# MLCogUP/nspeech

Measured on AMD Instinct MI355X. Metric: mel-frames/sec Tacotron-2 LJSpeech bs32 train step, higher is better.
Workload: dtype bf16; 1 GPU; Tacotron-2 train step (fwd+bwd+clip+Adam), batch 32/GPU, T_in 160, T_out 1000, r=5; targets = spectrogram features of synthetic speech (SURVEY 8d); global_batch=32, parallelism=dp1, deterministic_gradients=True

## Files before the change

### include/nspeech_hip.h

```cpp
#ifndef NSPEECH_HIP_H
#define NSPEECH_HIP_H
#include <stddef.h>
#include <stdint.h>

#ifdef __cplusplus
extern "C" {
#endif

typedef void* ns_stream_t;

enum { NS_OK = 0, NS_ERR_BAD_ARG = -1, NS_ERR_UNSUPPORTED_SHAPE = -2, NS_ERR_LAUNCH = -3,
       NS_ERR_SHORT_BUFFER = -4  };
enum { NS_F32 = 0, NS_BF16 = 1, NS_F64 = 2  };
enum { NS_ACT_NONE = 0, NS_ACT_RELU = 1, NS_ACT_TANH = 2, NS_ACT_SIGMOID = 3,
       NS_ACT_SOFTSIGN = 4  };

int ns_version(void);
const char* ns_device_arch(void);
const char* ns_last_error(void);

int ns_occupy(int blocks, int threads, int lds_bytes, int heavy, double usec, int* started, ns_stream_t stream);
int ns_wait_counter(const int* counter, int target, double timeout_usec, ns_stream_t stream);

typedef struct {
  float count, eps, momentum;
  int training;
  float* moving_mean; float* moving_var;
  float* mean_out; float* istd_out;
} ns_gemm_bn_params;
typedef struct {
  int dtype;
  int M, N, K;
  const void* A; int64_t lda; int a_mode;
  const void* B; int64_t ldb; int b_mode;
  int b_seg_len; int64_t b_seg_stride;
  void* C; int64_t ldc; int c_dtype;
  int accumulate;
  const float* bias;
  int act;
  float alpha;
  int row_period, row_lo, row_hi, row_shift;
  float* col_sum; float* col_sumsq;
  int split_k;
  const void* addend; int64_t ld_add;
  const void* gate; int64_t ld_gate;
  int f32_passes;
  int addend_dtype;
  const void* A_lo; const void* B_lo;
  int batch; int64_t batch_stride_a, batch_stride_b, batch_stride_c;
  float* stat_part;
  int stat_slots;
  const void* stat_z; int64_t ld_stat_z; int stat_z_dtype;
  const float* stat_mean; const float* stat_istd;
  float* splitk_work; int* splitk_count;
  ns_gemm_bn_params bn;
} ns_gemm_params;
int ns_gemm(const ns_gemm_params* p, ns_stream_t stream);
size_t ns_gemm_stat_part_floats(int M, int N);
size_t ns_gemm_splitk_work_bytes(int M, int N, int split_k);
size_t ns_gemm_splitk_counters(int M, int N);
const char* ns_gemm_last_kernel(void);



typedef struct {
  const void* src; int src_dtype; int64_t src_si, src_sj;
  void* dst; int dst_dtype; int64_t dst_si, dst_sj;
  int I, J, Cc;
  int accumulate;
} ns_copy3d_params;
int ns_copy3d(const ns_copy3d_params* p, ns_stream_t stream);

typedef struct {
  const int* ids;
  const float* table;
  void* out; int out_dtype;
  int N, T, P, padl, D, V;
} ns_embedding_params;
int ns_embedding_fwd(const ns_embedding_params* p, ns_stream_t stream);
typedef struct {
  const int* ids;
  const float* dout;
  float* dtable;
  int N, T, P, padl, D, V;
  float* work;
} ns_embedding_bwd_params;
int ns_embedding_bwd(const ns_embedding_bwd_params* p, ns_stream_t stream);
size_t ns_embedding_bwd_work_floats(int N, int D, int V);

typedef struct {
  const void* z; void* y; int dtype;
  int rows, C;
  const float* col_sum; const float* col_sumsq; float count;
  const float* gamma; const float* beta;
  float* moving_mean; float* moving_var;
  float* mean_out; float* istd_out;
  float eps, momentum;
  int training;
  int row_period, row_lo, row_hi;
  void* y_hi; void* y_lo;
  int64_t ld_y;
  int stats_final;
} ns_bn_fwd_params;
int ns_bn_fwd(const ns_bn_fwd_params* p, ns_stream_t stream);

typedef struct {
  const float* dy; const void* z; void* dpre; int dtype;
  int rows, C;
  const float* mean; const float* istd; const float* gamma;
  float* dgamma; float* dbeta; float* dbias;
  float* work;
  float count;
  int act;
  int row_period, row_lo, row_hi;
// ... 491 lines not shown
```

### nspeech_amd/csrc/gemm.hip

```cpp
#include "common.h"
#include "colsum4.h"
#include <limits.h>

struct Epi {
  void* C; long ldc; int c_dtype; int accumulate;
  const float* bias; int act; float alpha;
  int row_period, row_lo, row_hi, row_shift;
  int M, N;
  const void* addend; long ld_add; int add_bf16;
  const void* gate; long ld_gate; int gate_dtype;
  const void* sz; long ld_sz; int sz_bf16; const float* smean; const float* sistd;
};

__device__ __forceinline__ Epi make_epi(const ns_gemm_params& p) {
  Epi e;
  e.C = p.C; e.ldc = p.ldc; e.c_dtype = p.c_dtype; e.accumulate = p.accumulate;
  e.bias = p.bias; e.act = p.act; e.alpha = p.alpha;
  e.row_period = p.row_period; e.row_lo = p.row_lo; e.row_hi = p.row_hi; e.row_shift = p.row_shift;
  e.M = p.M; e.N = p.N;
  e.addend = p.addend; e.ld_add = p.ld_add; e.add_bf16 = p.addend_dtype == NS_BF16;
  e.gate = p.gate; e.ld_gate = p.ld_gate; e.gate_dtype = p.dtype;
  e.sz = p.stat_z; e.ld_sz = p.ld_stat_z; e.sz_bf16 = p.stat_z_dtype == NS_BF16; e.smean = p.stat_mean; e.sistd = p.stat_istd;
  return e;
}
// ... 197 lines not shown
    for (int j = 0; j < 4; ++j) { As[ty][tx * 4 + j] = s1[j]; Bs[ty][tx * 4 + j] = s2[j]; }
    __syncthreads();
    if (tid < BN && n0 + tid < p.N) {
      float a = 0.f, b = 0.f;
      for (int r = 0; r < 16; ++r) { a += As[r][tid]; b += Bs[r][tid]; }
      p.stat_part[(long)blockIdx.y * p.N + n0 + tid] = a;
      p.stat_part[((long)p.stat_slots + blockIdx.y) * p.N + n0 + tid] = b;
    }
  }
}

__global__ __launch_bounds__(1024) void gemm_stats_finalize_kernel(const float* part, int slots, int N, float* col_sum,
                                                                   float* col_sumsq, ns_gemm_bn_params bn) {
  __shared__ float red[32][33][2];
  const int c = threadIdx.x & 31, q = threadIdx.x >> 5;
  const int n = blockIdx.x * 32 + c;
  float a = 0.f, b = 0.f;
  if (n < N) {
    for (int s = q; s < slots; s += 32) {
      a += part[(long)s * N + n];
      b += part[((long)slots + s) * N + n];
    }
  }
  red[q][c][0] = a; red[q][c][1] = b;
  __syncthreads();
#pragma unroll
  for (int h = 16; h >= 1; h >>= 1) {
    if (q < h) { red[q][c][0] += red[q + h][c][0]; red[q][c][1] += red[q + h][c][1]; }
    __syncthreads();
  }
  if (q == 0 && n < N) {
    col_sum[n] = red[0][c][0];
    if (col_sumsq) col_sumsq[n] = red[0][c][1];
    if (bn.mean_out)
      bn_finalize_column(n, red[0][c][0], red[0][c][1], bn.count, bn.eps, bn.momentum, bn.training, bn.moving_mean,
                         bn.moving_var, bn.mean_out, bn.istd_out);
  }
}

constexpr int GBM = 128, GBN = 128, GBK = 64;

__device__ __forceinline__ int row_img_off(int row, int chunk) {
  return row * 128 + ((chunk ^ ((row >> 1) & 7)) << 4);
}
__device__ __forceinline__ int col_swz(int k) { return (k & 3) | ((k >> 1) & 4); }
__device__ __forceinline__ int col_img_off_chunk(int k, int chunk) {
  return k * 256 + ((chunk ^ (col_swz(k) << 1)) << 4);
}
__device__ __forceinline__ int col_img_off_unit(int k, int unit) {
  return k * 256 + ((unit ^ (col_swz(k) << 2)) << 3);
}

typedef __attribute__((address_space(3))) bf16x4 lds_bf16x4;

__device__ __forceinline__ bf16x8 frag_row(const char* img, int row, int chunk) {
  return *(const bf16x8*)(img + row_img_off(row, chunk));
}
__device__ __forceinline__ bf16x8 frag_col(const char* img, int kbase, int col0, int lane) {
  const int i16 = lane & 15, g = lane >> 4;
  const int q = i16 >> 2, pp = i16 & 3;
  const int k = kbase + 8 * g + q;
  const int unit = (col0 >> 2) + pp;
  bf16x4 t0 = __builtin_amdgcn_ds_read_tr16_b64_v4bf16((lds_bf16x4*)(img + col_img_off_unit(k, unit)));
  bf16x4 t1 = __builtin_amdgcn_ds_read_tr16_b64_v4bf16((lds_bf16x4*)(img + col_img_off_unit(k + 4, unit)));
  return __builtin_shufflevector(t0, t1, 0, 1, 2, 3, 4, 5, 6, 7);
}

struct Stage { uint4 v[4]; };

template <int MODE, int BK = GBK, int ROWS = 128>
__device__ __forceinline__ void stage_load(Stage& s, const bf16_t* base, long ld, int r0, int extent,
                                           int k0, int K, int tid) {
  if (MODE == 0) {
    const int c = tid & 7;
#pragma unroll
    for (int i = 0; i < ROWS / 32; ++i) {
      const int row = (tid >> 3) + 32 * i;
      const int r = r0 + row, k = k0 + c * 8;
      if (r < extent && k < K) s.v[i] = *(const uint4*)(base + (long)r * ld + k);
      else s.v[i] = make_uint4(0, 0, 0, 0);
    }
  } else {
    const int c = tid & 15;
#pragma unroll
    for (int i = 0; i < BK / 16; ++i) {
      const int kr = (tid >> 4) + 16 * i;
      const int k = k0 + kr, r = r0 + c * 8;
      if (k < K && r < extent) s.v[i] = *(const uint4*)(base + (long)k * ld + r);
      else s.v[i] = make_uint4(0, 0, 0, 0);
    }
  }
}
template <int MODE, int BK = GBK, int ROWS = 128>
__device__ __forceinline__ void stage_store(const Stage& s, char* img, int tid) {
  if (MODE == 0) {
    const int c = tid & 7;
#pragma unroll
    for (int i = 0; i < ROWS / 32; ++i) {
      const int row = (tid >> 3) + 32 * i;
      *(uint4*)(img + row_img_off(row, c)) = s.v[i];
    }
  } else {
    const int c = tid & 15;
#pragma unroll
    for (int i = 0; i < BK / 16; ++i) {
      const int kr = (tid >> 4) + 16 * i;
// ... 197 lines not shown
    char* imgB = imgA + IMG;
    const bool more = kt + 1 < kt1;
    if (more) {
      int kin;
      const bf16_t* bb = b_tile_base((kt + 1) * BK, kin);
      stage_load<AMODE, BK, TM>(sa, A, p.lda, m0, p.M, (kt + 1) * BK, p.K, tid);
      stage_load<BMODE, BK>(sb, bb, p.ldb, n0, p.N, kin, KB, tid);
    }
#pragma unroll
    for (int ks = 0; ks < BK / 32; ++ks) {
      bf16x8 af[4], bfr[NJ];
#pragma unroll
      for (int i = 0; i < 4; ++i) {
        if (AMODE == 0) af[i] = frag_row(imgA, wm * 64 + i * 16 + (lane & 15), ks * 4 + (lane >> 4));
        else af[i] = frag_col(imgA, ks * 32, wm * 64 + i * 16, lane);
      }
#pragma unroll
      for (int j = 0; j < NJ; ++j) {
        if (BMODE == 0) bfr[j] = frag_row(imgB, wn * (NJ * 16) + j * 16 + (lane & 15), ks * 4 + (lane >> 4));
        else bfr[j] = frag_col(imgB, ks * 32, wn * (NJ * 16) + j * 16, lane);
      }
#pragma unroll
      for (int i = 0; i < 4; ++i)
#pragma unroll
        for (int j = 0; j < NJ; ++j)
          acc[i][j] = VEC ? __builtin_amdgcn_mfma_f32_16x16x32_bf16(bfr[j], af[i], acc[i][j], 0, 0, 0)
                          : __builtin_amdgcn_mfma_f32_16x16x32_bf16(af[i], bfr[j], acc[i][j], 0, 0, 0);
    }
    if (more) {
      char* nA = smem + (cur ^ 1) * 2 * IMG;
      stage_store<AMODE, BK, TM>(sa, nA, tid);
      stage_store<BMODE, BK>(sb, nA + IMG, tid);
    }
    __syncthreads();
  }

  bool add_bias = ksl == 0;
  if (p.splitk_work && p.split_k > 1) {
    if (!splitk_gather_acc<NJ>(p, acc, wgid, ksl, tid)) return;
    add_bias = true;
  }
  if constexpr (VEC) x256_quadrant(p, acc, m0 + wm * 64, n0 + wn * (NJ * 16), lane);
  else mfma_epilogue(p, acc, m0, n0, wm, wn, lane, add_bias);
}
template <int AMODE, int BMODE, bool VEC, int BK = GBK, int TM = GBM>
__global__ __launch_bounds__(256, BK == 64 ? 2 : 3) void gemm_mfma_kernel(ns_gemm_params p) {
  const int nwg = ((p.M + TM - 1) / TM) * ((p.N + GBN - 1) / GBN);
  int wgid, ksl;
  xcd_work_item(p, nwg, wgid, ksl);
  batch_shift(p, blockIdx.z);
  gemm_mfma_body<AMODE, BMODE, VEC, BK, TM>(p, wgid, ksl);
}

constexpr int XHALF = 16384, XBUF = 65536;

typedef __attribute__((address_space(1))) const void* gptr_t;
typedef __attribute__((address_space(3))) void* lptr_t;

template <int NSEG>
__global__ __launch_bounds__(512, 1) void gemm_x256_kernel(ns_gemm_params p) {
  extern __shared__ __attribute__((aligned(1024))) char smem[];
  const int tid = threadIdx.x, lane = tid & 63;
  const int wave = __builtin_amdgcn_readfirstlane(tid >> 6);
  const int wr = wave >> 2, wc = wave & 3;
  const int tiles_n = (p.N + 255) / 256, tiles_m = (p.M + 255) / 256;
  const int nwg = tiles_m * tiles_n;
  int wgid;
  {
    const int orig = blockIdx.x, xcd = orig & 7, q = nwg >> 3, r = nwg & 7;
    wgid = (xcd < r ? xcd * (q + 1) : r * (q + 1) + (xcd - r) * q) + (orig >> 3);
  }
  const int tm = wgid / tiles_n, tn = wgid % tiles_n;
  const int m0 = tm * 256, n0 = tn * 256;
  const int nk = p.K / 64, NT = nk * NSEG;

  unsigned offA00, offA01, offA10, offA11, offB00, offB01, offB10, offB11;
  {
    const int r0 = wave * 8 + (lane >> 3), r1 = r0 + 64;
    const int c0 = (lane & 7) ^ ((r0 >> 1) & 7), c1 = (lane & 7) ^ ((r1 >> 1) & 7);
    auto oa = [&](int h, int r, int c) { return (unsigned)(((long)min(m0 + h * 128 + r, p.M - 1) * p.lda + c * 8) * 2); };
    auto ob = [&](int h, int r, int c) { return (unsigned)(((long)min(n0 + h * 128 + r, p.N - 1) * p.ldb + c * 8) * 2); };
    offA00 = oa(0, r0, c0); offA01 = oa(0, r1, c1); offA10 = oa(1, r0, c0); offA11 = oa(1, r1, c1);
    offB00 = ob(0, r0, c0); offB01 = ob(0, r1, c1); offB10 = ob(1, r0, c0); offB11 = ob(1, r1, c1);
  }
  const char* const Ahi = (const char*)p.A;
  const char* const Bhi = (const char*)p.B;
  const char* const Alo = (const char*)p.A_lo;
  const char* const Blo = (const char*)p.B_lo;
  char* const lstage = smem + wave * 1024;

#define X_ISSUE(T, HALF, O0, O1, ISA)                                                                   \
  do {                                                                                                   \
    const int t_ = (T);                                                                                  \
    if (t_ < NT) {                                                                                       \
      const int sg_ = NSEG == 1 ? 0 : t_ / nk;                                                           \
      const int kt_ = NSEG == 1 ? t_ : t_ - sg_ * nk;                                                    \
      const char* g_ = (ISA) ? (sg_ == NSEG - 1 && NSEG > 1 ? Alo : Ahi) : (sg_ == 1 && NSEG == 3 ? Blo : Bhi); \
      if (!(ISA) && p.b_seg_len > 0) {       \
        const int bs_ = (kt_ * 64) / p.b_seg_len;                                                        \
        g_ += ((long)bs_ * p.b_seg_stride + (kt_ * 64 - bs_ * p.b_seg_len)) * 2;                         \
      } else {                                                                                           \
        g_ += (long)kt_ * 128;                                                                           \
      }                                                                                                  \
      char* l_ = lstage + (t_ & 1) * XBUF + (HALF) * XHALF;                                              \
      __builtin_amdgcn_global_load_lds((gptr_t)(g_ + (O0)), (lptr_t)l_, 16, 0, 0);                       \
      __builtin_amdgcn_global_load_lds((gptr_t)(g_ + (O1)), (lptr_t)(l_ + 8192), 16, 0, 0);             \
    }                                                                                                    \
  } while (0)
#define X_ISSUE_A0(T) X_ISSUE(T, 0, offA00, offA01, 1)
#define X_ISSUE_A1(T) X_ISSUE(T, 1, offA10, offA11, 1)
// ... 370 lines not shown

template <int PASSES, int MT, int NC>
__global__ __launch_bounds__(SKW * 64) void gemm_skinny_f32_kernel(ns_gemm_params p) {
  __shared__ float red[SKW][16 * MT][20];
  const int tid = threadIdx.x, lane = tid & 63, wave = tid >> 6;
  const int n0 = blockIdx.x * NC;
  const int m0 = blockIdx.y * 16 * MT;
  const float* A = (const float*)p.A;
  const float* B = (const float*)p.B;
  const int r16 = lane & 15, g = lane >> 4;
  f32x4 acc[MT];
#pragma unroll
  for (int i = 0; i < MT; ++i) acc[i] = (f32x4){0.f, 0.f, 0.f, 0.f};
  const int nkc = (p.K + 31) / 32;
  const bool ok0 = m0 + r16 < p.M, ok1 = MT > 1 && m0 + 16 + r16 < p.M, okn = r16 < NC && n0 + r16 < p.N;
  for (int kc0 = wave; kc0 < nkc; kc0 += SKW * 2) {
    bf16x8 ah[2][MT], al[2][MT], bh[2], bl[2];
#pragma unroll
    for (int q = 0; q < 2; ++q) {
      const int k = (kc0 + q * SKW) * 32 + g * 8;
      const bool okk = k < p.K;
      ldsplit8(A + (long)(m0 + r16) * p.lda + k, ok0 && okk, ah[q][0], al[q][0]);
      if (MT > 1) ldsplit8(A + (long)(m0 + 16 + r16) * p.lda + k, ok1 && okk, ah[q][MT - 1], al[q][MT - 1]);
      ldsplit8(B + (long)(n0 + r16) * p.ldb + k, okn && okk, bh[q], bl[q]);
    }
#pragma unroll
    for (int q = 0; q < 2; ++q)
#pragma unroll
      for (int i = 0; i < MT; ++i) acc[i] = mfma_split<PASSES>(ah[q][i], al[q][i], bh[q], bl[q], acc[i]);
  }
#pragma unroll
  for (int i = 0; i < MT; ++i)
#pragma unroll
    for (int r = 0; r < 4; ++r) red[wave][i * 16 + g * 4 + r][r16] = acc[i][r];
  __syncthreads();
  Epi e = make_epi(p);
  for (int idx = tid; idx < 16 * MT * NC; idx += SKW * 64) {
    const int mm = idx / NC, nn = idx % NC;
    const int m = m0 + mm, n = n0 + nn;
    if (m >= p.M || n >= p.N) continue;
    float v = 0.f;
#pragma unroll
    for (int w = 0; w < SKW; ++w) v += red[w][mm][nn];
    const bool valid = row_valid(e, m);
    v = epi_value(e, m, n, v, true, valid);
    epi_store(e, m, n, v);
  }
}

static bool aligned16(const void* p) { return (((uintptr_t)p) & 15) == 0; }

static thread_local const char* g_last_kernel = "";
extern "C" const char* ns_gemm_last_kernel(void) { return g_last_kernel; }

static bool vec_epilogue_ok(const ns_gemm_params& p) {
  auto al = [](const void* q, long ld, bool bf16) { return !q || ((((uintptr_t)q) & (bf16 ? 7 : 15)) == 0 && ld % 4 == 0); };
  if (p.accumulate == 2 || p.split_k != 1 || p.N % 4 != 0) return false;
  if (p.batch > 1 && p.batch_stride_c % 4 != 0) return false;
  return al(p.C, p.ldc, p.c_dtype == NS_BF16) && al(p.addend, p.ld_add, p.addend_dtype == NS_BF16) &&
         al(p.gate, p.ld_gate, p.dtype == NS_BF16) && al(p.stat_z, p.ld_stat_z, p.stat_z_dtype == NS_BF16) &&
         al(p.bias, 4, false) && al(p.stat_mean, 4, false) && al(p.stat_istd, 4, false) && al(p.stat_part, 4, false);
}
static bool half_tiles_wanted(const ns_gemm_params& p, int tiles128) {
  static const int env = [] { const char* e = getenv("NS_GEMM_HALF"); return e ? atoi(e) : -1; }();
  if (env == 0 || env == 1) return env != 0;
  return tiles128 * p.batch <= (env > 1 ? env : 256) && p.M > 64;
}
static bool x256_ok(const ns_gemm_params& p) {
  if (p.dtype != NS_BF16 || p.a_mode != 0 || p.b_mode != 0 || p.split_k != 1) return false;
  if (p.b_seg_len != 0 && (p.b_seg_len % 64 != 0 || p.b_seg_stride % 8 != 0)) return false;
  if (p.K % 64 != 0 || p.K < 128 || p.M < 1024 || p.N % 128 != 0) return false;
  if ((p.A_lo != nullptr) != (p.B_lo != nullptr)) return false;
  if (p.A_lo && (!aligned16(p.A_lo) || !aligned16(p.B_lo))) return false;
  {
    auto al = [](const void* q, long ld, bool bf16) { return !q || ((((uintptr_t)q) & (bf16 ? 7 : 15)) == 0 && ld % 4 == 0); };
    if (!al(p.C, p.ldc, p.c_dtype == NS_BF16) || !al(p.addend, p.ld_add, p.addend_dtype == NS_BF16) ||
        !al(p.gate, p.ld_gate, true) || !al(p.stat_z, p.ld_stat_z, p.stat_z_dtype == NS_BF16) || !al(p.bias, 4, false) ||
        !al(p.stat_mean, 4, false) || !al(p.stat_istd, 4, false) || !al(p.stat_part, 4, false)) return false;
  }
  if ((double)p.M * (double)p.lda * 2.0 >= 4.0e9 || (double)p.N * (double)p.ldb * 2.0 >= 4.0e9) return false;
  if (getenv("NS_GEMM_NO256")) return false;
  return ceil_div(p.M, 256) * ceil_div(p.N, 256) >= 96;
}

extern "C" size_t ns_gemm_stat_part_floats(int M, int N) {
  if (M <= 0 || N <= 0) return 0;
  return (size_t)2 * 4 * ceil_div(M, 256) * (size_t)N;
}

static int gemm_dispatch(ns_gemm_params& p, hipStream_t stream);

int ns_stats_finalize(const float* part, int slots, int N, float* s1, float* s2, hipStream_t stream) {
  hipLaunchKernelGGL(gemm_stats_finalize_kernel, dim3(ceil_div(N, 32)), dim3(1024), 0, stream, part, slots, N, s1, s2,
                     ns_gemm_bn_params{});
  NS_CHECK_LAUNCH("gemm_stats_finalize");
  return NS_OK;
}

extern "C" size_t ns_gemm_splitk_work_bytes(int M, int N, int split_k) {
  if (split_k <= 1) return 0;
  return (size_t)split_k * ((size_t)ceil_div(M, 128) * 128) * ((size_t)ceil_div(N, 128) * 128) * sizeof(float);
}
extern "C" size_t ns_gemm_splitk_counters(int M, int N) { return (size_t)ceil_div(M, 64) * ceil_div(N, 64); }

extern "C" int ns_gemm(const ns_gemm_params* pp, ns_stream_t stream_) {
  hipStream_t stream = (hipStream_t)stream_;
// ... 16 lines not shown
  p.stat_slots = 0;
  int rc = gemm_dispatch(p, stream);
  if (rc || !p.stat_part || p.M == 0 || p.N == 0) return rc;
  hipLaunchKernelGGL(gemm_stats_finalize_kernel, dim3(ceil_div(p.N, 32)), dim3(1024), 0, stream, p.stat_part, p.stat_slots,
                     p.N, p.col_sum, p.col_sumsq, bn);
  NS_CHECK_LAUNCH("gemm_stats_finalize");
  return NS_OK;
}

static int gemm_normalize(ns_gemm_params& p) {
  NS_CHECK_ARG(p.A && p.B && p.C, "ns_gemm: null operand");
  NS_CHECK_ARG(p.dtype == NS_F32 || p.dtype == NS_BF16, "ns_gemm: bad dtype %d", p.dtype);
  NS_CHECK_ARG(p.c_dtype == NS_F32 || p.c_dtype == NS_BF16, "ns_gemm: bad c_dtype %d", p.c_dtype);
  if (p.split_k < 1) p.split_k = 1;
  NS_CHECK_ARG((p.splitk_work != nullptr) == (p.splitk_count != nullptr), "ns_gemm: splitk_work and splitk_count come together");
  NS_CHECK_ARG(!p.splitk_work || p.split_k == 1 || p.batch <= 1, "ns_gemm: deterministic split-K takes no batch");
  NS_CHECK_ARG(!p.splitk_work || ns_gemm_splitk_work_bytes(p.M, p.N, p.split_k) < 0x7ffffff0ull,
               "ns_gemm: deterministic split-K scratch beyond 2 GB (32-bit buffer offsets): lower split_k");
  NS_CHECK_ARG(p.accumulate >= 0 && p.accumulate <= 2, "ns_gemm: bad accumulate");
  NS_CHECK_ARG(p.accumulate == 0 || p.c_dtype == NS_F32, "ns_gemm: accumulate needs fp32 C");
  NS_CHECK_ARG(p.split_k == 1 || (p.accumulate == 2 && p.act == NS_ACT_NONE && !p.col_sum),
               "ns_gemm: split_k>1 needs atomic accumulate, no activation, no stats");
  NS_CHECK_ARG(p.b_seg_len == 0 || (p.b_seg_len > 0 && p.K % p.b_seg_len == 0),
               "ns_gemm: K must be a multiple of b_seg_len");
  NS_CHECK_ARG(p.dtype != NS_F32 || p.f32_passes == 0 || p.f32_passes == 1 || p.f32_passes == 3,
               "ns_gemm: f32_passes = %d on fp32 operands (0, 1 or 3; 2 is the two-segment product of pre-split bf16 operands)",
               p.f32_passes);
  if (p.alpha == 0.f) p.alpha = 1.f;
  if (p.batch < 1) p.batch = 1;
  NS_CHECK_ARG(p.batch == 1 || (!p.col_sum && !p.bias && !p.addend && !p.gate && !p.A_lo && p.batch <= 65535),
               "ns_gemm: batched calls take no bias / addend / gate / statistics / pre-split operands");
  return NS_OK;
}

enum { GF_SKINNY, GF_X256, GF_PRESPLIT_REFUSED, GF_MFMA, GF_SKINNY_F32, GF_F32, GF_GENERIC };
struct gemm_form { int kind; bool vec, half, bk32; };
static gemm_form gemm_classify(const ns_gemm_params& p) {
  bool fast = (p.dtype == NS_BF16) && aligned16(p.A) && aligned16(p.B) && (p.lda % 8 == 0) &&
              (p.ldb % 8 == 0) && (p.b_seg_stride % 8 == 0) && (p.batch_stride_a % 8 == 0) &&
              (p.batch_stride_b % 8 == 0);
  if (fast) {
    if (p.a_mode == 0) fast = fast && (p.K % 8 == 0); else fast = fast && (p.M % 8 == 0);
    if (p.b_mode == 0) fast = fast && (p.K % 8 == 0); else fast = fast && (p.N % 8 == 0);
    if (p.b_seg_len > 0) fast = fast && (p.b_seg_len % GBK == 0);
  }
  if (fast && p.M <= 32 && p.a_mode == 0 && p.b_mode == 0 && p.b_seg_len == 0 && p.split_k == 1 &&
      !p.col_sum && p.batch == 1 && !p.A_lo && !p.B_lo) return {GF_SKINNY, false, false, false};
  if (fast && p.batch == 1 && x256_ok(p)) return {GF_X256, false, false, false};
  if (p.A_lo || p.B_lo) return {GF_PRESPLIT_REFUSED, false, false, false};
  if (fast) {
    const int tiles = ceil_div(p.M, GBM) * ceil_div(p.N, GBN);
    const bool vec = vec_epilogue_ok(p);
    const bool half = vec && p.a_mode == 0 && half_tiles_wanted(p, tiles);
    static const int bk32_env = [] { const char* e = getenv("NS_GEMM_BK32"); return e ? atoi(e) : -1; }();
    const bool bk32w = bk32_env >= 0 ? bk32_env != 0 : (long)tiles * p.split_k * p.batch >= 600;
    const bool bk32 = !half && p.a_mode == 1 && p.b_mode == 1 && bk32w && (p.b_seg_len == 0 || p.b_seg_len % 32 == 0);
    return {GF_MFMA, vec, half, bk32};
  }
  if (p.dtype == NS_F32 && p.f32_passes > 0) {
    bool ok = aligned16(p.A) && aligned16(p.B) && (p.lda % 4 == 0) && (p.ldb % 4 == 0) && (p.b_seg_stride % 4 == 0) &&
              (p.batch_stride_a % 4 == 0) && (p.batch_stride_b % 4 == 0);
    if (p.a_mode == 0) ok = ok && (p.K % 4 == 0); else ok = ok && (p.M % 4 == 0);
    if (p.b_mode == 0) ok = ok && (p.K % 4 == 0); else ok = ok && (p.N % 4 == 0);
    if (p.b_seg_len > 0) ok = ok && (p.b_seg_len % FBK == 0);
    if (ok && p.M <= 32 && p.a_mode == 0 && p.b_mode == 0 && p.b_seg_len == 0 && p.split_k == 1 && !p.col_sum &&
        p.K % 8 == 0 && p.lda % 4 == 0 && p.batch == 1) return {GF_SKINNY_F32, false, false, false};
    if (ok) {
      const int tiles = ceil_div(p.M, GBM) * ceil_div(p.N, GBN);
      const bool vec = vec_epilogue_ok(p);
      return {GF_F32, vec, vec && p.a_mode == 0 && half_tiles_wanted(p, tiles), false};
    }
  }
  return {GF_GENERIC, false, false, false};
}

static int gemm_dispatch(ns_gemm_params& p, hipStream_t stream) {
  NS_CHECK_ARG(p.M >= 0 && p.N >= 0 && p.K >= 0, "ns_gemm: negative dims");
  if (p.M == 0 || p.N == 0) return NS_OK;
  if (int rc = gemm_normalize(p)) return rc;
  const gemm_form form = gemm_classify(p);
  if (form.kind == GF_SKINNY) {
    g_last_kernel = p.N >= 32 * 128 ? "gemm_skinny_kernel<2>" : "gemm_skinny_kernel<1>";
    if (p.N >= 32 * 128) hipLaunchKernelGGL(gemm_skinny_kernel<2>, dim3(ceil_div(p.N, 32)), dim3(SKW * 64), 0, stream, p);
    else hipLaunchKernelGGL(gemm_skinny_kernel<1>, dim3(ceil_div(p.N, 16)), dim3(SKW * 64), 0, stream, p);
    NS_CHECK_LAUNCH("gemm_skinny");
    return NS_OK;
  }
  if (form.kind == GF_X256) {
    const int tiles = ceil_div(p.M, 256) * ceil_div(p.N, 256);
    const size_t lds = 2 * XBUF;
    static bool attr_set = false;
    if (!attr_set) {
      (void)hipFuncSetAttribute((const void*)gemm_x256_kernel<1>, hipFuncAttributeMaxDynamicSharedMemorySize, (int)lds);
      (void)hipFuncSetAttribute((const void*)gemm_x256_kernel<3>, hipFuncAttributeMaxDynamicSharedMemorySize, (int)lds);
      (void)hipFuncSetAttribute((const void*)gemm_x256_kernel<2>, hipFuncAttributeMaxDynamicSharedMemorySize, (int)lds);
      attr_set = true;
    }
    p.stat_slots = 4 * ceil_div(p.M, 256);
    const bool two = p.A_lo && p.f32_passes == 2;
    g_last_kernel = p.A_lo ? (two ? "gemm_x256_kernel<2>" : "gemm_x256_kernel<3>") : "gemm_x256_kernel<1>";
    if (two) hipLaunchKernelGGL(gemm_x256_kernel<2>, dim3(tiles), dim3(512), lds, stream, p);
    else if (p.A_lo) hipLaunchKernelGGL(gemm_x256_kernel<3>, dim3(tiles), dim3(512), lds, stream, p);
    else hipLaunchKernelGGL(gemm_x256_kernel<1>, dim3(tiles), dim3(512), lds, stream, p);
    NS_CHECK_LAUNCH("gemm_x256");
    return NS_OK;
  }
  NS_CHECK_ARG(form.kind != GF_PRESPLIT_REFUSED, "ns_gemm: pre-split operands (A_lo / B_lo) need the 256-tile path "
               "(bf16, a_mode 0, b_mode 0, K %% 64 == 0, M >= 1024, N %% 128 == 0, >= 96 tiles, no split_k)");
  if (form.kind == GF_MFMA) {
    const int tiles = ceil_div(p.M, GBM) * ceil_div(p.N, GBN);
    dim3 grid(tiles, p.split_k, p.batch);
    const size_t lds = 65536;
    p.stat_slots = 2 * ceil_div(p.M, GBM);
    const bool vec = form.vec, half = form.half;
    if (half) {
      grid.x = ceil_div(p.M, 64) * ceil_div(p.N, GBN);
      p.stat_slots = ceil_div(p.M, 64);
    }
#define LAUNCH_MFMA(AM, BM_)                                                                      \
  do {                                                                                            \
    static bool attr_set = false;                                                                 \
    if (!attr_set) {                                                                              \
      (void)hipFuncSetAttribute((const void*)gemm_mfma_kernel<AM, BM_, false>,                        \
                          hipFuncAttributeMaxDynamicSharedMemorySize, (int)lds);                  \
      (void)hipFuncSetAttribute((const void*)gemm_mfma_kernel<AM, BM_, true>,                         \
                          hipFuncAttributeMaxDynamicSharedMemorySize, (int)lds);                  \
      attr_set = true;                                                                            \
    }                                                                                             \
    g_last_kernel = vec ? "gemm_mfma_kernel<" #AM ", " #BM_ ", true, 64, 128>" : "gemm_mfma_kernel<" #AM ", " #BM_ ", false, 64, 128>";  \
    if (vec) hipLaunchKernelGGL((gemm_mfma_kernel<AM, BM_, true>), grid, dim3(256), lds, stream, p);  \
    else hipLaunchKernelGGL((gemm_mfma_kernel<AM, BM_, false>), grid, dim3(256), lds, stream, p);     \
  } while (0)
#define LAUNCH_MFMA_HALF(BM_)                                                                     \
  do {                                                                                            \
    static bool attr_set = false;                                                                 \
    if (!attr_set) {                                                                              \
      (void)hipFuncSetAttribute((const void*)gemm_mfma_kernel<0, BM_, true, 64, 64>,                  \
                          hipFuncAttributeMaxDynamicSharedMemorySize, (int)lds);                  \
      attr_set = true;                                                                            \
    }                                                                                             \
    g_last_kernel = "gemm_mfma_kernel<0, " #BM_ ", true, 64, 64>";                                \
    hipLaunchKernelGGL((gemm_mfma_kernel<0, BM_, true, 64, 64>), grid, dim3(256), lds, stream, p);    \
  } while (0)
    if (half) {
      if (p.b_mode == 0) LAUNCH_MFMA_HALF(0); else LAUNCH_MFMA_HALF(1);
    } else if (form.bk32) {
      g_last_kernel = vec ? "gemm_mfma_kernel<1, 1, true, 32, 128>" : "gemm_mfma_kernel<1, 1, false, 32, 128>";
      if (vec) hipLaunchKernelGGL((gemm_mfma_kernel<1, 1, true, 32>), grid, dim3(256), 32768, stream, p);
      else hipLaunchKernelGGL((gemm_mfma_kernel<1, 1, false, 32>), grid, dim3(256), 32768, stream, p);
    } else if (p.a_mode == 0 && p.b_mode == 0) LAUNCH_MFMA(0, 0);
    else if (p.a_mode == 0 && p.b_mode == 1) LAUNCH_MFMA(0, 1);
    else if (p.a_mode == 1 && p.b_mode == 0) LAUNCH_MFMA(1, 0);
    else LAUNCH_MFMA(1, 1);
#undef LAUNCH_MFMA_HALF
#undef LAUNCH_MFMA
    NS_CHECK_LAUNCH("gemm_mfma");
    return NS_OK;
  }
  if (form.kind == GF_SKINNY_F32 || form.kind == GF_F32) {
    const bool three = p.f32_passes >= 3;
    if (form.kind == GF_SKINNY_F32) {
      if (ceil_div(p.N, 16) <= 64) {
        g_last_kernel = three ? "gemm_skinny_f32_kernel<3, 1, 8>" : "gemm_skinny_f32_kernel<1, 1, 8>";
        const dim3 grid(ceil_div(p.N, 8), ceil_div(p.M, 16));
        if (three) hipLaunchKernelGGL((gemm_skinny_f32_kernel<3, 1, 8>), grid, dim3(SKW * 64), 0, stream, p);
        else hipLaunchKernelGGL((gemm_skinny_f32_kernel<1, 1, 8>), grid, dim3(SKW * 64), 0, stream, p);
      } else {
        g_last_kernel = three ? "gemm_skinny_f32_kernel<3, 2, 16>" : "gemm_skinny_f32_kernel<1, 2, 16>";
        if (three) hipLaunchKernelGGL((gemm_skinny_f32_kernel<3, 2, 16>), dim3(ceil_div(p.N, 16)), dim3(SKW * 64), 0, stream, p);
        else hipLaunchKernelGGL((gemm_skinny_f32_kernel<1, 2, 16>), dim3(ceil_div(p.N, 16)), dim3(SKW * 64), 0, stream, p);
      }
      NS_CHECK_LAUNCH("gemm_skinny_f32");
      return NS_OK;
    }
    {
      const int tiles = ceil_div(p.M, GBM) * ceil_div(p.N, GBN);
      dim3 grid(tiles, p.split_k, p.batch);
      const size_t lds = 65536;
      p.stat_slots = 2 * ceil_div(p.M, GBM);
      const bool vec = form.vec, half = form.half;
      if (half) {
        grid.x = ceil_div(p.M, 64) * ceil_div(p.N, GBN);
        p.stat_slots = ceil_div(p.M, 64);
      }
#define LAUNCH_F32(AM, BM_, PS)                                                                     \
  do {                                                                                              \
    static bool attr_set = false;                                                                   \
    if (!attr_set) {                                                                                \
      (void)hipFuncSetAttribute((const void*)gemm_mfma_f32_kernel<AM, BM_, PS, false>,              \
                                hipFuncAttributeMaxDynamicSharedMemorySize, (int)lds);              \
      (void)hipFuncSetAttribute((const void*)gemm_mfma_f32_kernel<AM, BM_, PS, true>,               \
                                hipFuncAttributeMaxDynamicSharedMemorySize, (int)lds);              \
      attr_set = true;                                                                              \
    }                                                                                               \
    g_last_kernel = vec ? "gemm_mfma_f32_kernel<" #AM ", " #BM_ ", " #PS ", true, 128>"             \
                        : "gemm_mfma_f32_kernel<" #AM ", " #BM_ ", " #PS ", false, 128>";           \
    if (vec) hipLaunchKernelGGL((gemm_mfma_f32_kernel<AM, BM_, PS, true>), grid, dim3(256), lds, stream, p);   \
    else hipLaunchKernelGGL((gemm_mfma_f32_kernel<AM, BM_, PS, false>), grid, dim3(256), lds, stream, p);      \
  } while (0)
#define LAUNCH_F32_HALF(BM_, PS)                                                                    \
  do {                                                                                              \
    static bool attr_set = false;                                                                   \
    if (!attr_set) {                                                                                \
      (void)hipFuncSetAttribute((const void*)gemm_mfma_f32_kernel<0, BM_, PS, true, 64>,            \
                                hipFuncAttributeMaxDynamicSharedMemorySize, (int)lds);              \
      attr_set = true;                                                                              \
    }                                                                                               \
    g_last_kernel = "gemm_mfma_f32_kernel<0, " #BM_ ", " #PS ", true, 64>";                         \
    hipLaunchKernelGGL((gemm_mfma_f32_kernel<0, BM_, PS, true, 64>), grid, dim3(256), lds, stream, p);         \
  } while (0)
#define LAUNCH_F32_MODES(PS)                                                   \
  do {                                                                         \
    if (half && p.b_mode == 0) LAUNCH_F32_HALF(0, PS);                         \
    else if (half) LAUNCH_F32_HALF(1, PS);                                     \
    else if (p.a_mode == 0 && p.b_mode == 0) LAUNCH_F32(0, 0, PS);             \
    else if (p.a_mode == 0 && p.b_mode == 1) LAUNCH_F32(0, 1, PS);             \
    else if (p.a_mode == 1 && p.b_mode == 0) LAUNCH_F32(1, 0, PS);             \
    else LAUNCH_F32(1, 1, PS);                                                 \
  } while (0)
      if (three) LAUNCH_F32_MODES(3); else LAUNCH_F32_MODES(1);
#undef LAUNCH_F32_HALF
#undef LAUNCH_F32_MODES
#undef LAUNCH_F32
      NS_CHECK_LAUNCH("gemm_mfma_f32");
      return NS_OK;
    }
  }
  dim3 grid(ceil_div(p.N, 64), ceil_div(p.M, 64), p.split_k * p.batch);
  p.stat_slots = ceil_div(p.M, 64);
  g_last_kernel = "gemm_generic_kernel";
  if (p.dtype == NS_F32) hipLaunchKernelGGL(gemm_generic_kernel<float>, grid, dim3(256), 0, stream, p);
  else hipLaunchKernelGGL(gemm_generic_kernel<bf16_t>, grid, dim3(256), 0, stream, p);
  NS_CHECK_LAUNCH("gemm_generic");
  return NS_OK;
}

struct gemm_group_args {
  int wg0[NS_GEMM_GROUP_MAX];
  ns_gemm_group_item item[NS_GEMM_GROUP_MAX];
};
static_assert(sizeof(ns_gemm_group_item) == 112, "ns_gemm_group_item: layout of include/nspeech_hip.h");
static_assert(sizeof(gemm_group_args) <= 4096, "the item table must fit the kernel argument block");
extern "C" size_t ns_gemm_group_arg_bytes(void) { return sizeof(gemm_group_args); }

__device__ __forceinline__ ns_gemm_params group_product(const ns_gemm_group_item& it) {
  ns_gemm_params p = {};
  p.dtype = it.dtype;
  p.M = it.M; p.N = it.N; p.K = it.K;
  p.A = it.A; p.lda = it.lda; p.a_mode = 1;
  p.B = it.B; p.ldb = it.ldb; p.b_mode = 1;
  p.b_seg_len = it.b_seg_len; p.b_seg_stride = it.b_seg_stride;
  p.C = it.C; p.ldc = it.ldc; p.c_dtype = NS_F32;
  p.accumulate = 2;
  p.alpha = 1.f;
  p.split_k = it.split_k;
  p.f32_passes = 1;
  p.batch = 1;
  p.splitk_work = it.work; p.splitk_count = it.count;
  return p;
}

__global__ __launch_bounds__(256, 2) void gemm_group_kernel(const gemm_group_args a) {
  extern __shared__ __attribute__((aligned(16))) char smem[];
  const int b = blockIdx.x;
  int idx = 0;
#pragma unroll
  for (int i = 1; i < NS_GEMM_GROUP_MAX; ++i) idx += b >= a.wg0[i];
  const ns_gemm_group_item& it = a.item[idx];
  const int local = b - it.wg0;
  if (local >= it.nwg) return;
  if (it.kind == 2) {
    ns_colsum_params c;
    c.x = it.A; c.dtype = it.dtype; c.ld = it.lda; c.rows = it.K; c.C = it.N; c.out = (float*)it.C; c.work = it.work;
    const int gx = colsum4_grid_x(c.rows);
    float (*red)[4] = (float (*)[4])smem;
    int* last = (int*)(smem + 256 * 4 * sizeof(float));
    if (it.dtype == NS_BF16) colsum4_body<bf16_t>(c, local % gx, local / gx, gx, red, last);
    else colsum4_body<float>(c, local % gx, local / gx, gx, red, last);
    return;
  }
  const ns_gemm_params p = group_product(it);
  const int tiles = ((it.M + GBM - 1) / GBM) * ((it.N + GBN - 1) / GBN);
  int tile, ksl;
  xcd_group_item(it.split_k, tiles, local, tile, ksl);
  if (it.kind == 0) gemm_mfma_body<1, 1, false, GBK, GBM>(p, tile, ksl);
  else gemm_mfma_f32_body<1, 1, 1, false, GBM>(p, tile, ksl);
}

namespace {
struct group_entry {
  ns_gemm_group_item it;
  int index, k_extent;
  const char* c0; const char* c1;
  const char* s0[2]; const char* s1[2];
};
bool ranges_meet(const char* a0, const char* a1, const char* b0, const char* b1) { return a0 < b1 && b0 < a1 && a0 < a1 && b0 < b1; }
}

static int gemm_group_build(const ns_gemm_params* products, int n_products, const ns_colsum_params* sums, int n_sums,
                            group_entry* out, int* n_out) {
  NS_CHECK_ARG(n_products >= 0 && n_sums >= 0 && n_products + n_sums > 0, "ns_gemm_group: empty list");
  NS_CHECK_ARG((n_products == 0 || products) && (n_sums == 0 || sums), "ns_gemm_group: null list");
  int n = 0;
  for (int i = 0; i < n_products; ++i) {
    ns_gemm_params p = products[i];
    NS_CHECK_ARG(p.M >= 0 && p.N >= 0 && p.K >= 0, "ns_gemm_group: product %d: negative dims", i);
    group_entry e = {};
    e.index = i;
    e.it.kind = p.dtype == NS_F32 ? 1 : 0;
    if (p.M > 0 && p.N > 0) {
      if (int rc = gemm_normalize(p)) return rc;
      NS_CHECK_ARG(p.accumulate == 2 && p.alpha == 1.f && p.c_dtype == NS_F32 && p.batch == 1,
                   "ns_gemm_group: product %d: items are atomic fp32 accumulations (accumulate 2, alpha 1, batch 1)", i);
      NS_CHECK_ARG(!p.bias && p.act == NS_ACT_NONE && !p.gate && !p.addend && !p.col_sum && !p.col_sumsq && !p.stat_z &&
                   p.row_period <= 0 && !p.A_lo && !p.B_lo && !p.bn.mean_out,
                   "ns_gemm_group: product %d carries an epilogue operand the item table has no field for", i);
      const gemm_form f = gemm_classify(p);
      const bool k0 = f.kind == GF_MFMA && !f.vec && !f.half && !f.bk32;
      const bool k1 = f.kind == GF_F32 && !f.vec && !f.half && p.f32_passes == 1;
      NS_CHECK_ARG((k0 || k1) && p.a_mode == 1 && p.b_mode == 1,
                   "ns_gemm_group: product %d is not one ns_gemm runs on gemm_mfma_kernel<1, 1, false, 64, 128> or "
                   "gemm_mfma_f32_kernel<1, 1, 1, false, 128>", i);
      const int tiles = ceil_div(p.M, GBM) * ceil_div(p.N, GBN);
      const int bk = k0 ? GBK : FBK, nk = ceil_div(p.K, bk), per = ceil_div(nk, p.split_k);
      ns_gemm_group_item& it = e.it;
      it.A = p.A; it.B = p.B; it.C = p.C; it.work = p.split_k > 1 ? p.splitk_work : nullptr;
      it.count = p.split_k > 1 ? p.splitk_count : nullptr;
      it.lda = p.lda; it.ldb = p.ldb; it.ldc = p.ldc; it.b_seg_stride = p.b_seg_stride;
      it.M = p.M; it.N = p.N; it.K = p.K; it.b_seg_len = p.b_seg_len;
      it.split_k = p.split_k; it.dtype = p.dtype; it.kind = k0 ? 0 : 1;
      it.nwg = tiles * p.split_k;
      e.k_extent = min((long)p.K, (long)per * bk);
      e.c0 = (const char*)p.C; e.c1 = e.c0 + ((long)(p.M - 1) * p.ldc + p.N) * 4;
      if (it.work) {
        e.s0[0] = (const char*)it.work; e.s1[0] = e.s0[0] + ns_gemm_splitk_work_bytes(p.M, p.N, p.split_k);
        e.s0[1] = (const char*)it.count; e.s1[1] = e.s0[1] + (size_t)tiles * 4;
      }
    }
    out[n++] = e;
// ... 34 lines not shown
    for (; j > 0 && out[j - 1].k_extent < e.k_extent; --j) out[j] = out[j - 1];
    out[j] = e;
  }
  int in_launch = 0, wg = 0;
  for (int i = 0; i < n; ++i) {
    ns_gemm_group_item& it = out[i].it;
    if (it.nwg > 0 && in_launch == NS_GEMM_GROUP_MAX) { in_launch = 0; wg = 0; }
    it.wg0 = wg;
    it.reserved = 0;
    if (it.nwg > 0) { ++in_launch; wg = (wg + it.nwg + 7) & ~7; }
  }
  *n_out = n;
  return NS_OK;
}

static int group_launch_end(const group_entry* e, int n, int first) {
  int i = first, seen = 0;
  for (; i < n; ++i) {
    if (e[i].it.nwg > 0 && seen == NS_GEMM_GROUP_MAX) break;
    if (e[i].it.nwg > 0) ++seen;
  }
  return i;
}

extern "C" int ns_gemm_group_plan(const ns_gemm_params* products, int n_products, const ns_colsum_params* sums, int n_sums,
                                  ns_gemm_group_plan_entry* entries, int* n_launches) {
  if (n_launches) *n_launches = 0;
  NS_CHECK_ARG(n_products >= 0 && n_sums >= 0 && n_products + n_sums > 0, "ns_gemm_group: empty list");
  group_entry* e = new group_entry[n_products + n_sums];
  int n = 0;
  const int rc = gemm_group_build(products, n_products, sums, n_sums, e, &n);
  if (rc == NS_OK) {
    int launches = 0;
    for (int first = 0; first < n; ++launches) {
      const int end = group_launch_end(e, n, first);
      for (int i = first; i < end && entries; ++i)
        entries[i] = ns_gemm_group_plan_entry{e[i].index, e[i].it.kind, launches, e[i].it.wg0, e[i].it.nwg, e[i].k_extent};
      first = end;
    }
    if (n_launches) *n_launches = launches;
  }
  delete[] e;
  return rc;
}

extern "C" int ns_gemm_group(const ns_gemm_params* products, int n_products, const ns_colsum_params* sums, int n_sums,
                             ns_stream_t stream_) {
  NS_CHECK_ARG(n_products >= 0 && n_sums >= 0 && n_products + n_sums > 0, "ns_gemm_group: empty list");
  group_entry* e = new group_entry[n_products + n_sums];
  int n = 0;
  int rc = gemm_group_build(products, n_products, sums, n_sums, e, &n);
  static bool attr_set = false;
  if (rc == NS_OK && !attr_set) {
    (void)hipFuncSetAttribute((const void*)gemm_group_kernel, hipFuncAttributeMaxDynamicSharedMemorySize, 65536);
    attr_set = true;
  }
  for (int first = 0; rc == NS_OK && first < n;) {
    const int end = group_launch_end(e, n, first);
    gemm_group_args a;
    int k = 0, total = 0;
    for (int i = first; i < end; ++i) {
      if (e[i].it.nwg <= 0) continue;
      a.wg0[k] = e[i].it.wg0;
      a.item[k++] = e[i].it;
      total = e[i].it.wg0 + e[i].it.nwg;
    }
    for (int i = k; i < NS_GEMM_GROUP_MAX; ++i) { a.wg0[i] = INT_MAX; a.item[i] = ns_gemm_group_item{}; }
    if (k > 0) {
      g_last_kernel = "gemm_group_kernel";
      hipLaunchKernelGGL(gemm_group_kernel, dim3(total), dim3(256), 65536, (hipStream_t)stream_, a);
      if (hipGetLastError() != hipSuccess) { ns_set_error("gemm_group: launch failed"); rc = NS_ERR_LAUNCH; }
    }
    first = end;
  }
  delete[] e;
  return rc;
}
```

Before: 1.790 million mel-frames/s.

## Add direct-to-LDS buffer-load pipeline for MFMA GEMMs with both operands K-major

```diff
diff --git a/include/nspeech_hip.h b/include/nspeech_hip.h
--- a/include/nspeech_hip.h
+++ b/include/nspeech_hip.h
@@ -60,6 +60,7 @@
 size_t ns_gemm_splitk_work_bytes(int M, int N, int split_k);
 size_t ns_gemm_splitk_counters(int M, int N);
 const char* ns_gemm_last_kernel(void);
+const char* ns_gemm_last_loop(void);
 
 
 
diff --git a/nspeech_amd/csrc/gemm.hip b/nspeech_amd/csrc/gemm.hip
--- a/nspeech_amd/csrc/gemm.hip
+++ b/nspeech_amd/csrc/gemm.hip
@@ -273,6 +273,8 @@
 }
 
 typedef __attribute__((address_space(3))) bf16x4 lds_bf16x4;
+typedef __attribute__((address_space(1))) const void* gptr_t;
+typedef __attribute__((address_space(3))) void* lptr_t;
 
 __device__ __forceinline__ bf16x8 frag_row(const char* img, int row, int chunk) {
   return *(const bf16x8*)(img + row_img_off(row, chunk));
@@ -576,10 +578,135 @@
   gemm_mfma_body<AMODE, BMODE, VEC, BK, TM>(p, wgid, ksl);
 }
 
+typedef unsigned int dma_rsrc __attribute__((ext_vector_type(4)));
+__device__ __forceinline__ dma_rsrc dma_descriptor(const void* base, long bytes) {
+  const uintptr_t b = (uintptr_t)base;
+  return (dma_rsrc){(unsigned)__builtin_amdgcn_readfirstlane((int)(unsigned)b),
+                    (unsigned)__builtin_amdgcn_readfirstlane((int)((unsigned)(b >> 32) & 0xffffu)),
+                    (unsigned)__builtin_amdgcn_readfirstlane((int)bytes), 0x00020000u};
+}
+__device__ __forceinline__ void dma_load16(const dma_rsrc& rs, unsigned lds, unsigned voff) {
+  unsigned keep;
+  asm volatile("s_mov_b32 %0, m0\n\ts_mov_b32 m0, %1\n\ts_nop 0\n\tbuffer_load_dwordx4 %2, %3, 0 offen lds\n\ts_mov_b32 m0, %0"
+               : "=&s"(keep) : "s"(__builtin_amdgcn_readfirstlane((int)lds)), "v"(voff), "s"(rs) : "memory");
+}
+template <bool VEC, int BK, int NST>
+__device__ __forceinline__ void gemm_mfma_dma_body(const ns_gemm_params& p, const int wgid, const int ksl) {
+  constexpr int IMG = BK * 256;
+  constexpr int LPI = BK / 16;
+  constexpr int LPT = 2 * LPI;
+  static_assert(NST == 2 || NST == 3, "two or three tile buffers");
+  static_assert(NST * 2 * IMG * (BK == 64 ? 2 : 3) <= 160 * 1024, "the workgroups of a CU share 160 KB");
+  extern __shared__ __attribute__((aligned(16))) char smem[];
+  const int tid = threadIdx.x, lane = tid & 63;
+  const int wave = __builtin_amdgcn_readfirstlane(tid >> 6);
+  const int wm = wave >> 1, wn = wave & 1;
+  const int tiles_n = (p.N + GBN - 1) / GBN;
+  const int tm = wgid / tiles_n, tn = wgid % tiles_n;
+  const int m0 = tm * GBM, n0 = tn * GBN;
+
+  const int nk = (p.K + BK - 1) / BK;
+  const int per = (nk + p.split_k - 1) / p.split_k;
+  const int kt0 = ksl * per, kt1 = min(nk, kt0 + per);
+  const int nt = kt1 - kt0;
+
+  f32x4 acc[4][4];
+#pragma unroll
+  for (int i = 0; i < 4; ++i)
+#pragma unroll
+    for (int j = 0; j < 4; ++j) acc[i][j] = (f32x4){0.f, 0.f, 0.f, 0.f};
+
+  constexpr unsigned OUT = 0x80000000u;
+  const long b_rows = p.b_seg_len > 0 ? (long)(p.K / p.b_seg_len - 1) * p.b_seg_stride + (long)(p.b_seg_len - 1) * p.ldb
+                                      : (long)(p.K - 1) * p.ldb;
+  const dma_rsrc ra = dma_descriptor(p.A, ((long)(p.K - 1) * p.lda + p.M) * 2);
+  const dma_rsrc rb = dma_descriptor(p.B, (b_rows + p.N) * 2);
+  const int kr = tid >> 4;
+  const int ch = (tid & 15) ^ (col_swz(kr) << 1);
+  const unsigned lda2 = (unsigned)p.lda * 2u, ldb2 = (unsigned)p.ldb * 2u;
+  const unsigned a_lane = m0 + ch * 8 < p.M ? (unsigned)kr * lda2 + (unsigned)(m0 + ch * 8) * 2u : OUT;
+  const unsigned b_lane = n0 + ch * 8 < p.N ? (unsigned)kr * ldb2 + (unsigned)(n0 + ch * 8) * 2u : OUT;
+  const unsigned lpiece = (unsigned)(uintptr_t)(lptr_t)smem + wave * 1024;
+
+  auto issue = [&](int t, int buf) {
+    const int k0 = (kt0 + t) * BK;
+    const unsigned a_tile = (unsigned)k0 * lda2;
+    unsigned b_tile = (unsigned)k0 * ldb2;
+    if (p.b_seg_len > 0) {
+      const int s = k0 / p.b_seg_len;
+      b_tile = (unsigned)(((long)s * p.b_seg_stride + (long)(k0 - s * p.b_seg_len) * p.ldb) * 2);
+    }
+    const unsigned dst = lpiece + buf * 2 * IMG;
+    if (k0 + BK <= p.K) {
+#pragma unroll
+      for (int i = 0; i < LPI; ++i)
+        dma_load16(ra, dst + i * 4096, a_lane + a_tile + (unsigned)(16 * i) * lda2);
+#pragma unroll
+      for (int i = 0; i < LPI; ++i)
+        dma_load16(rb, dst + IMG + i * 4096, b_lane + b_tile + (unsigned)(16 * i) * ldb2);
+    } else {
+#pragma unroll
+      for (int i = 0; i < LPI; ++i) {
+        const bool in = k0 + 16 * i + kr < p.K;
+        dma_load16(ra, dst + i * 4096, in ? a_lane + a_tile + (unsigned)(16 * i) * lda2 : OUT);
+      }
+#pragma unroll
+      for (int i = 0; i < LPI; ++i) {
+        const bool in = k0 + 16 * i + kr < p.K;
+        dma_load16(rb, dst + IMG + i * 4096, in ? b_lane + b_tile + (unsigned)(16 * i) * ldb2 : OUT);
+      }
+    }
+  };
+
+#pragma unroll
+  for (int t = 0; t < NST - 1; ++t)
+    if (t < nt) issue(t, t);
+
+  int cur = 0;
+  for (int t = 0; t < nt; ++t) {
+    const int ahead = min(NST - 2, nt - 1 - t);
+    if (NST >= 3 && ahead == 1) asm volatile("s_waitcnt vmcnt(%0)" ::"n"(LPT) : "memory");
+    else asm volatile("s_waitcnt vmcnt(0)" ::: "memory");
+    __builtin_amdgcn_s_barrier();
+    asm volatile("" ::: "memory");
+    if (t + NST - 1 < nt) issue(t + NST - 1, cur == 0 ? NST - 1 : cur - 1);
+    const char* imgA = smem + cur * 2 * IMG;
+    const char* imgB = imgA + IMG;
+#pragma unroll
+    for (int ks = 0; ks < BK / 32; ++ks) {
+      bf16x8 af[4], bfr[4];
+#pragma unroll
+      for (int i = 0; i < 4; ++i) af[i] = frag_col(imgA, ks * 32, wm * 64 + i * 16, lane);
+#pragma unroll
+      for (int j = 0; j < 4; ++j) bfr[j] = frag_col(imgB, ks * 32, wn * 64 + j * 16, lane);
+#pragma unroll
+      for (int i = 0; i < 4; ++i)
+#pragma unroll
+        for (int j = 0; j < 4; ++j)
+          acc[i][j] = VEC ? __builtin_amdgcn_mfma_f32_16x16x32_bf16(bfr[j], af[i], acc[i][j], 0, 0, 0)
+                          : __builtin_amdgcn_mfma_f32_16x16x32_bf16(af[i], bfr[j], acc[i][j], 0, 0, 0);
+    }
+    cur = cur == NST - 1 ? 0 : cur + 1;
+  }
+
+  bool add_bias = ksl == 0;
+  if (p.splitk_work && p.split_k > 1) {
+    if (!splitk_gather_acc<4>(p, acc, wgid, ksl, tid)) return;
+    add_bias = true;
+  }
+  if constexpr (VEC) x256_quadrant(p, acc, m0 + wm * 64, n0 + wn * 64, lane);
+  else mfma_epilogue(p, acc, m0, n0, wm, wn, lane, add_bias);
+}
+template <bool VEC, int BK, int NST>
+__global__ __launch_bounds__(256, BK == 64 ? 2 : 3) void gemm_mfma_dma_kernel(ns_gemm_params p) {
+  const int nwg = ((p.M + GBM - 1) / GBM) * ((p.N + GBN - 1) / GBN);
+  int wgid, ksl;
+  xcd_work_item(p, nwg, wgid, ksl);
+  batch_shift(p, blockIdx.z);
+  gemm_mfma_dma_body<VEC, BK, NST>(p, wgid, ksl);
+}
+
 constexpr int XHALF = 16384, XBUF = 65536;
-
-typedef __attribute__((address_space(1))) const void* gptr_t;
-typedef __attribute__((address_space(3))) void* lptr_t;
 
 template <int NSEG>
 __global__ __launch_bounds__(512, 1) void gemm_x256_kernel(ns_gemm_params p) {
@@ -1056,6 +1183,19 @@
 
 static thread_local const char* g_last_kernel = "";
 extern "C" const char* ns_gemm_last_kernel(void) { return g_last_kernel; }
+static thread_local const char* g_last_loop = "staged";
+extern "C" const char* ns_gemm_last_loop(void) { return g_last_loop; }
+
+static bool gemm_dma_ok(const ns_gemm_params& p) {
+  const char* e = getenv("NS_GEMM_DMA");
+  if (e && atoi(e) == 0) return false;
+  if (p.a_mode != 1 || p.b_mode != 1 || p.K < 1 || p.lda < 0 || p.ldb < 0 || p.b_seg_stride < 0) return false;
+  const double a_bytes = ((double)(p.K - 1) * (double)p.lda + p.M) * 2.0;
+  const double b_bytes = p.b_seg_len > 0 ? ((double)(p.K / p.b_seg_len - 1) * (double)p.b_seg_stride +
+                                            (double)(p.b_seg_len - 1) * (double)p.ldb + p.N) * 2.0
+                                         : ((double)(p.K - 1) * (double)p.ldb + p.N) * 2.0;
+  return a_bytes < 2147483648.0 && b_bytes < 2147483648.0;
+}
 
 static bool vec_epilogue_ok(const ns_gemm_params& p) {
   auto al = [](const void* q, long ld, bool bf16) { return !q || ((((uintptr_t)q) & (bf16 ? 7 : 15)) == 0 && ld % 4 == 0); };
@@ -1178,7 +1318,8 @@
     const int tiles = ceil_div(p.M, GBM) * ceil_div(p.N, GBN);
     const bool vec = vec_epilogue_ok(p);
     const bool half = vec && p.a_mode == 0 && half_tiles_wanted(p, tiles);
-    static const int bk32_env = [] { const char* e = getenv("NS_GEMM_BK32"); return e ? atoi(e) : -1; }();
+    const char* const bk32_e = getenv("NS_GEMM_BK32");
+    const int bk32_env = bk32_e ? atoi(bk32_e) : -1;
     const bool bk32w = bk32_env >= 0 ? bk32_env != 0 : (long)tiles * p.split_k * p.batch >= 600;
     const bool bk32 = !half && p.a_mode == 1 && p.b_mode == 1 && bk32w && (p.b_seg_len == 0 || p.b_seg_len % 32 == 0);
     return {GF_MFMA, vec, half, bk32};
@@ -1205,6 +1346,7 @@
   if (p.M == 0 || p.N == 0) return NS_OK;
   if (int rc = gemm_normalize(p)) return rc;
   const gemm_form form = gemm_classify(p);
+  g_last_loop = "staged";
   if (form.kind == GF_SKINNY) {
     g_last_kernel = p.N >= 32 * 128 ? "gemm_skinny_kernel<2>" : "gemm_skinny_kernel<1>";
     if (p.N >= 32 * 128) hipLaunchKernelGGL(gemm_skinny_kernel<2>, dim3(ceil_div(p.N, 32)), dim3(SKW * 64), 0, stream, p);
@@ -1268,7 +1410,30 @@
     g_last_kernel = "gemm_mfma_kernel<0, " #BM_ ", true, 64, 64>";                                \
     hipLaunchKernelGGL((gemm_mfma_kernel<0, BM_, true, 64, 64>), grid, dim3(256), lds, stream, p);    \
   } while (0)
-    if (half) {
+#define LAUNCH_DMA(BK_, NST_)                                                                                  \
+  do {                                                                                                         \
+    static bool attr_set = false;                                                                              \
+    constexpr int lds_ = NST_ * BK_ * 512;                                                                     \
+    if (!attr_set) {                                                                                           \
+      (void)hipFuncSetAttribute((const void*)gemm_mfma_dma_kernel<false, BK_, NST_>,                           \
+                                hipFuncAttributeMaxDynamicSharedMemorySize, lds_);                             \
+      (void)hipFuncSetAttribute((const void*)gemm_mfma_dma_kernel<true, BK_, NST_>,                            \
+                                hipFuncAttributeMaxDynamicSharedMemorySize, lds_);                             \
+      attr_set = true;                                                                                         \
+    }                                                                                                          \
+    if (vec) hipLaunchKernelGGL((gemm_mfma_dma_kernel<true, BK_, NST_>), grid, dim3(256), lds_, stream, p);    \
+    else hipLaunchKernelGGL((gemm_mfma_dma_kernel<false, BK_, NST_>), grid, dim3(256), lds_, stream, p);       \
+  } while (0)
+    if (!half && p.a_mode == 1 && p.b_mode == 1 && gemm_dma_ok(p)) {
+      g_last_loop = "dma";
+      if (form.bk32) {
+        g_last_kernel = vec ? "gemm_mfma_kernel<1, 1, true, 32, 128>" : "gemm_mfma_kernel<1, 1, false, 32, 128>";
+        LAUNCH_DMA(32, 3);
+      } else {
+        g_last_kernel = vec ? "gemm_mfma_kernel<1, 1, true, 64, 128>" : "gemm_mfma_kernel<1, 1, false, 64, 128>";
+        LAUNCH_DMA(64, 2);
+      }
+    } else if (half) {
       if (p.b_mode == 0) LAUNCH_MFMA_HALF(0); else LAUNCH_MFMA_HALF(1);
     } else if (form.bk32) {
       g_last_kernel = vec ? "gemm_mfma_kernel<1, 1, true, 32, 128>" : "gemm_mfma_kernel<1, 1, false, 32, 128>";
@@ -1278,6 +1443,7 @@
     else if (p.a_mode == 0 && p.b_mode == 1) LAUNCH_MFMA(0, 1);
     else if (p.a_mode == 1 && p.b_mode == 0) LAUNCH_MFMA(1, 0);
     else LAUNCH_MFMA(1, 1);
+#undef LAUNCH_DMA
 #undef LAUNCH_MFMA_HALF
 #undef LAUNCH_MFMA
     NS_CHECK_LAUNCH("gemm_mfma");
@@ -1369,7 +1535,7 @@
 static_assert(sizeof(gemm_group_args) <= 4096, "the item table must fit the kernel argument block");
 extern "C" size_t ns_gemm_group_arg_bytes(void) { return sizeof(gemm_group_args); }
 
-__device__ __forceinline__ ns_gemm_params group_product(const ns_gemm_group_item& it) {
+__host__ __device__ __forceinline__ ns_gemm_params group_product(const ns_gemm_group_item& it) {
   ns_gemm_params p = {};
   p.dtype = it.dtype;
   p.M = it.M; p.N = it.N; p.K = it.K;
@@ -1386,6 +1552,7 @@
   return p;
 }
 
+template <bool DMA>
 __global__ __launch_bounds__(256, 2) void gemm_group_kernel(const gemm_group_args a) {
   extern __shared__ __attribute__((aligned(16))) char smem[];
   const int b = blockIdx.x;
@@ -1409,8 +1576,10 @@
   const int tiles = ((it.M + GBM - 1) / GBM) * ((it.N + GBN - 1) / GBN);
   int tile, ksl;
   xcd_group_item(it.split_k, tiles, local, tile, ksl);
-  if (it.kind == 0) gemm_mfma_body<1, 1, false, GBK, GBM>(p, tile, ksl);
-  else gemm_mfma_f32_body<1, 1, 1, false, GBM>(p, tile, ksl);
+  if (it.kind == 0) {
+    if constexpr (DMA) gemm_mfma_dma_body<false, GBK, 2>(p, tile, ksl);
+    else gemm_mfma_body<1, 1, false, GBK, GBM>(p, tile, ksl);
+  } else gemm_mfma_f32_body<1, 1, 1, false, GBM>(p, tile, ksl);
 }
 
 namespace {
@@ -1551,15 +1720,18 @@
   int rc = gemm_group_build(products, n_products, sums, n_sums, e, &n);
   static bool attr_set = false;
   if (rc == NS_OK && !attr_set) {
-    (void)hipFuncSetAttribute((const void*)gemm_group_kernel, hipFuncAttributeMaxDynamicSharedMemorySize, 65536);
+    (void)hipFuncSetAttribute((const void*)gemm_group_kernel<false>, hipFuncAttributeMaxDynamicSharedMemorySize, 65536);
+    (void)hipFuncSetAttribute((const void*)gemm_group_kernel<true>, hipFuncAttributeMaxDynamicSharedMemorySize, 65536);
     attr_set = true;
   }
   for (int first = 0; rc == NS_OK && first < n;) {
     const int end = group_launch_end(e, n, first);
     gemm_group_args a;
     int k = 0, total = 0;
+    bool dma = true;
     for (int i = first; i < end; ++i) {
       if (e[i].it.nwg <= 0) continue;
+      if (e[i].it.kind == 0) dma = dma && gemm_dma_ok(group_product(e[i].it));
       a.wg0[k] = e[i].it.wg0;
       a.item[k++] = e[i].it;
       total = e[i].it.wg0 + e[i].it.nwg;
@@ -1567,7 +1739,9 @@
     for (int i = k; i < NS_GEMM_GROUP_MAX; ++i) { a.wg0[i] = INT_MAX; a.item[i] = ns_gemm_group_item{}; }
     if (k > 0) {
       g_last_kernel = "gemm_group_kernel";
-      hipLaunchKernelGGL(gemm_group_kernel, dim3(total), dim3(256), 65536, (hipStream_t)stream_, a);
+      g_last_loop = dma ? "dma" : "staged";
+      if (dma) hipLaunchKernelGGL(gemm_group_kernel<true>, dim3(total), dim3(256), 65536, (hipStream_t)stream_, a);
+      else hipLaunchKernelGGL(gemm_group_kernel<false>, dim3(total), dim3(256), 65536, (hipStream_t)stream_, a);
       if (hipGetLastError() != hipSuccess) { ns_set_error("gemm_group: launch failed"); rc = NS_ERR_LAUNCH; }
     }
     first = end;
```

Measured after the change: 1.816 million mel-frames/s, median of 6. 1.4% higher.
